# chenjiaoAngel/Paddle-Lite

Measured on AMD Instinct MI355X. Metric: INT8 images/sec MobileNetV1 224x224, higher is better.
Workload: dtype int8; 1 GPU; MobileNetV1 INT8 full graph 224x224 (27 int8 convs + pool + fc + softmax), random-init weights, 128 images per step and GPU (4 predictors / HIP streams, each running whole steps: 4 steps in flight), input resident in HBM; steps_in_flight=4, global_batch=128

## Files before the change

### paddle-lite_amd/csrc/fused_dwpw_stream.hip

```cpp
#include <stdlib.h>

#include <type_traits>

#include "plhip_device.h"
#include "plhip_kernels.h"
#include "dw_common.h"
#include "gemm_tr_common.h"

namespace plhip {

typedef float v2f __attribute__((ext_vector_type(2)));


constexpr int FS_STAMP_SLOTS = 8;

template <int W, int K, int M, int TP, int RS, int PD, int S, int MP, int OUT, bool DWNN, bool PWNN>
__global__ __launch_bounds__(256, M / MP >= 256 ? 2 : 3) void fused_dwpw_stream_kernel(FusedArgs a) {
  constexpr int FS_TP = TP, FS_NT = TP / 32, FS_PITCH = fs_pitch(TP);
  static_assert((FS_PITCH / 4) % 16 == 8 && FS_PITCH >= TP, "image pitch");
  constexpr int RP = (W + 3) / 4 * 4;
  constexpr int TR = W == 14 ? 7 : FS_TP / RP, NS = TR / RS, QW = RP / 4;
  static_assert(RP == W || (S == 2 && RP == 16), "partial quads: the stride-2 form only");
  constexpr int G = 64 / QW;
  constexpr int NGRP = K * NS;
  constexpr int NIT = (NGRP + 4 * G - 1) / (4 * G);
  constexpr int KS = K / 32, MT = M / 32 / MP;
  constexpr int MSPLIT = MT >= 4 ? 4 : MT;
  constexpr int NSPLIT = 4 / MSPLIT;
  constexpr int MW = MT / MSPLIT;
  constexpr int NW = (FS_NT + NSPLIT - 1) / NSPLIT;
  constexpr int NIN = S == 1 ? RS + 2 : 2 * RS + 1;
  constexpr int ND = S == 1 ? 2 : 3;
  constexpr int WI = S * W;
  static_assert(S == 1 || S == 2, "stride");
  static_assert(TR * RP <= FS_TP && TR % RS == 0 && K % 32 == 0 && M % (32 * MP) == 0 && MT % MSPLIT == 0, "geometry");
  const GemmArgs& g = a.pw;
  PLHIP_PRELOAD(a.x); PLHIP_PRELOAD(a.dw_w); PLHIP_PRELOAD(a.dw_scale); PLHIP_PRELOAD(a.dw_bias); PLHIP_PRELOAD(a.dw_act);
  PLHIP_PRELOAD(a.dw_alpha); PLHIP_PRELOAD(a.n); PLHIP_PRELOAD(a.h); PLHIP_PRELOAD(a.tiles); PLHIP_PRELOAD(a.ones); PLHIP_PRELOAD(g.wp);
  PLHIP_PRELOAD(g.y); PLHIP_PRELOAD(g.scale); PLHIP_PRELOAD(g.bias); PLHIP_PRELOAD(g.act); PLHIP_PRELOAD(g.alpha); PLHIP_PRELOAD(g.NT);
  extern __shared__ __attribute__((aligned(16))) uint8_t fs_lds[];
  const int lane = threadIdx.x & 63;
  const int wave = __builtin_amdgcn_readfirstlane(threadIdx.x >> 6);
  const unsigned nb = (unsigned)a.tiles, per = (nb + 7) >> 3;
  const unsigned vb = (blockIdx.x & 7) * per + (blockIdx.x >> 3);
  if (vb >= nb) return;
  const int H = a.oh, TPI = g.NT;
  const int b = (int)(vb / (unsigned)TPI), ti = (int)(vb - (unsigned)b * TPI), tr0 = ti * TR;
  const int c = lane & 31, h = lane >> 5;
  unsigned long long* const gstamp = PLHIP_STAMPS_OF(g);
  const bool diag = kStamps && gstamp && vb < 2048;
  unsigned long long* const lstamp = diag ? gstamp + ((size_t)vb * 4 + wave) * FS_STAMP_SLOTS : nullptr;
  PLHIP_STAMP_REAL(0);
  PLHIP_STAMP(1);

  const int gl = lane / QW, q = lane - gl * QW;
  const bool active = gl < G;
  const int colq = q == 0 ? 0 : (q == QW - 1 ? W - 8 : 4 * q - 1);
  const uint32_t sel_lo = q == 0 ? 0x0201000cu : (q == QW - 1 ? 0x06050403u : 0x03020100u);
  const uint32_t sel_hi = q == 0 ? 0x06050403u : (q == QW - 1 ? 0x0c0c0c07u : 0x07060504u);
  const float dw_hi2 = a.dw_act == ACT_RELU6 ? fminf(a.dw_alpha + a.dw_alpha, 254.f) : 254.f;
  const float dw_leak = a.dw_act == ACT_LEAKY ? a.dw_alpha : 1.f;
  const uint32_t plane = (uint32_t)H * W, plane_in = (uint32_t)a.h * WI;
  const uint32_t m0 = q == 0 ? 0xffffff00u : 0xffffffffu;
  constexpr bool OVER = RP > W;
  const int x_last = (int)((uint32_t)a.n * K * plane_in) - 12;

  uint32_t in[PD][NIN][ND];
  uint8_t* const prm = fs_lds + (size_t)K * FS_PITCH;
  static_assert(K <= 256, "one channel's parameters per thread");
  uint32_t pw0 = 0, pw1 = 0, pw2 = 0;
  float psc0 = 0.f, pbi0 = 0.f;
  if ((int)threadIdx.x < K) {
    const int8_t* wp = a.dw_w + (size_t)threadIdx.x * 9;
    __builtin_memcpy(&pw0, wp, 4);
    __builtin_memcpy(&pw1, wp + 3, 4);
    __builtin_memcpy(&pw2, wp + 5, 4);
    psc0 = a.dw_scale[threadIdx.x];
    pbi0 = (a.dw_bias ? a.dw_bias : a.dw_scale)[threadIdx.x];
  }
  auto task = [&](int it, int& ch, int& strip, int& r0) {
    int gi = (it * 4 + wave) * G + (active ? gl : 0);
    if (gi >= NGRP) gi = NGRP - 1;
    ch = gi / NS;
    strip = gi - ch * NS;
    r0 = tr0 + strip * RS;
    if (r0 > H - RS) r0 = H - RS;
  };
  using std::integral_constant;
  auto fetch = [&](auto it_c) __attribute__((always_inline)) {
    constexpr int it = decltype(it_c)::value, s = it % PD;
    int ch, strip, r0;
    task(it, ch, strip, r0);
    const uint8_t* xs = reinterpret_cast<const uint8_t*>(a.x);
    if constexpr (S == 1) {
      const uint32_t off0 = (uint32_t)(b * K + ch) * plane + (uint32_t)r0 * W + colq;
      const bool top = r0 == 0, bot = r0 + RS == H;
      __builtin_memcpy(in[s][0], xs + (top ? off0 : off0 - W), 8);
#pragma unroll
      for (int t = 1; t <= RS; ++t) __builtin_memcpy(in[s][t], xs + off0 + (t - 1) * W, 8);
      __builtin_memcpy(in[s][RS + 1], xs + (bot ? off0 + (RS - 1) * W : off0 + RS * W), 8);
    } else {
      const int off0 = (int)((uint32_t)(b * K + ch) * plane_in + (uint32_t)(2 * r0) * WI) + 8 * q - 4;
      const int o1 = off0 < 0 ? 0 : off0;
      __builtin_memcpy(in[s][0], xs + (r0 == 0 ? o1 : off0 - WI), 12);
      __builtin_memcpy(in[s][1], xs + o1, 12);
#pragma unroll
      for (int t = 2; t < NIN; ++t) {
        int o = off0 + (t - 1) * WI;
        if (OVER && t == NIN - 1) o = o > x_last ? x_last : o;
        __builtin_memcpy(in[s][t], xs + o, 12);
      }
    }
  };
  auto compute = [&](auto it_c) __attribute__((always_inline)) {
    constexpr int it = decltype(it_c)::value, s = it % PD;
    int ch, strip, r0;
    task(it, ch, strip, r0);
    const uint32_t zt = r0 == 0 ? 0u : 0xffffffffu, zb = r0 + RS == H ? 0u : 0xffffffffu;
    constexpr bool SINK = M / MP < 256;
    const uint32_t ldsa = (uint32_t)ch * FS_PITCH + (uint32_t)(strip * RS) * RP + 4 * q;
    const uint32_t ldsw = SINK && !active ? (uint32_t)(K * FS_PITCH + K * 32) + 4 * (lane & 7) : ldsa;
    int dacc[RS][4];
    const v4i pv = *reinterpret_cast<const v4i*>(prm + ch * 32);
    const uint32_t wr[3] = {(uint32_t)pv[0], (uint32_t)pv[1], (uint32_t)pv[2]};
    const uint32_t w0t = wr[0] & zt, w2b = S == 1 ? wr[2] & zb : wr[2];
    const uint32_t wu[3] = {wr[0] << 8, wr[1] << 8, wr[2] << 8};
    const uint32_t w0tu = w0t << 8;
    const bool fix = S == 2 && b == 0 && ch == 0 && q == 0 && r0 == 0;
    const bool fixe = OVER && b == a.n - 1 && ch == K - 1 && q == QW - 1 && r0 + RS == H;
    const float dsc = __uint_as_float((uint32_t)pv[3]), dbi = __uint_as_float(*reinterpret_cast<const uint32_t*>(prm + ch * 32 + 16));
#pragma unroll
    for (int t = 0; t < NIN; ++t) {
      uint32_t win[4];
      if constexpr (S == 1) {
        const uint32_t e0 = __builtin_amdgcn_perm(in[s][t][1], in[s][t][0], sel_lo), e1 = __builtin_amdgcn_perm(in[s][t][1], in[s][t][0], sel_hi);
        win[0] = e0;
        win[1] = __builtin_amdgcn_alignbyte(e1, e0, 1);
        win[2] = __builtin_amdgcn_alignbyte(e1, e0, 2);
        win[3] = __builtin_amdgcn_alignbyte(e1, e0, 3);
#pragma unroll
        for (int r = 0; r < 3; ++r) {
          const int o = t - r;
          if (o < 0 || o >= RS) continue;
#pragma unroll
          for (int jj = 0; jj < 4; ++jj)
            dacc[o][jj] = r == 0 ? sdot4_first(win[jj], t == 0 ? w0t : wr[0])
                                 : __builtin_amdgcn_sdot4((int)win[jj], (int)(t == NIN - 1 ? w2b : wr[r]), dacc[o][jj], false);
        }
      } else {
        uint32_t d0 = in[s][t][0], d1 = in[s][t][1], d2 = in[s][t][2];
        if (t < 2) {
          d2 = fix ? d1 : d2;
          d1 = fix ? d0 : d1;
        }
        if (OVER && t == NIN - 1) {
          d0 = fixe ? d1 : d0;
          d1 = fixe ? d2 : d1;
        }
        win[0] = __builtin_amdgcn_alignbyte(d1, d0, 3) & m0;
        win[1] = __builtin_amdgcn_alignbyte(d2, d1, 1);
        win[2] = __builtin_amdgcn_alignbyte(d2, d1, 3);
        win[3] = d2;
#pragma unroll
        for (int r = 0; r < 3; ++r) {
          if ((t - r) & 1) continue;
          const int o = (t - r) / 2;
          if (t - r < 0 || o >= RS) continue;
          const uint32_t f = t == 0 ? w0t : wr[r], fu = t == 0 ? w0tu : wu[r];
#pragma unroll
          for (int jj = 0; jj < 4; ++jj)
            dacc[o][jj] = r == 0 ? sdot4_first(win[jj], jj == 3 ? fu : f)
                                 : __builtin_amdgcn_sdot4((int)win[jj], (int)(jj == 3 ? fu : f), dacc[o][jj], false);
        }
      }
    }
#pragma unroll
    for (int o = 0; o < RS; ++o) {
      const uint32_t pk = DWNN ? requant4_nn_rtz(dacc[o], dsc, dbi, dw_hi2, a.ones)
                               : dw_requant4<ACT_LEAKY>(dacc[o], dsc, dbi, dw_leak, -254.f, 254.f);
      if (SINK || active) *reinterpret_cast<uint32_t*>(fs_lds + ldsw + o * RP) = pk;
    }
  };
  auto prime = [&](auto self, auto it_c) __attribute__((always_inline)) -> void {
    constexpr int it = decltype(it_c)::value;
    if constexpr (it < PD && it < NIT) {
      fetch(it_c);
      self(self, integral_constant<int, it + 1>{});
    }
  };
  prime(prime, integral_constant<int, 0>{});
  PLHIP_STAMP(2);
  const int ms = wave % MSPLIT, ns = wave / MSPLIT;
  const int n0 = ns * NW;
  const int nmine = n0 + NW <= FS_NT ? NW : FS_NT - n0;
  const uint32_t trb = (uint32_t)(((h * 2) * 8 + ((lane & 15) >> 1)) * FS_PITCH + ((lane >> 4) & 1) * 16 + (lane & 1) * 8 + n0 * 32);
  const uint32_t wlane = (uint32_t)lane * 16;
  constexpr int WBUDGET = 192, ACCR = NW * MW * 16;
  constexpr int WD = KS < 4 ? 2 : (ACCR + KS * MW * 4 <= WBUDGET ? KS : (ACCR + 4 * MW * 4 <= WBUDGET ? 4 : 2));
  constexpr int WPRE = WD == KS ? KS : WD - 1;
  constexpr bool ALOOK = M / MP >= 256 && NSPLIT == 1 && ACCR + WD * MW * 4 <= WBUDGET;
  v4i Wf[WD][MW];
  float psc[2][MW], pbi[2][MW];
  auto pass_w = [&](int mp) { return reinterpret_cast<const uint8_t*>(g.wp) + (size_t)((mp * MSPLIT + ms) * MW) * KS * 1024; };
  auto pass_operands = [&](auto mp_c) __attribute__((always_inline)) {
    constexpr int mp = decltype(mp_c)::value;
    const uint8_t* const wpk = pass_w(mp);
    const int mt0 = (mp * MSPLIT + ms) * MW;
#pragma unroll
    for (int u = 0; u < WPRE && u < KS; ++u)
#pragma unroll
      for (int m = 0; m < MW; ++m) Wf[u][m] = *reinterpret_cast<const v4i*>(wpk + ((size_t)m * KS + u) * 1024 + wlane);
#pragma unroll
    for (int m = 0; m < MW; ++m) {
      psc[mp & 1][m] = 1.f;
      pbi[mp & 1][m] = 0.f;
      if (OUT != OUT_I32) {
        psc[mp & 1][m] = g.scale[(mt0 + m) * 32 + c];
        pbi[mp & 1][m] = (g.bias ? g.bias : g.scale)[(mt0 + m) * 32 + c];
        if (!g.bias) pbi[mp & 1][m] = 0.f;
      }
    }
  };
  pass_operands(integral_constant<int, 0>{});
  if ((int)threadIdx.x < K) {
    uint32_t* o = reinterpret_cast<uint32_t*>(prm + threadIdx.x * 32);
    const v4i pv = {(int)(pw0 & 0xffffffu), (int)(pw1 & 0xffffffu), (int)(pw2 >> 8), (int)__float_as_uint(psc0 + psc0)};
    *reinterpret_cast<v4i*>(o) = pv;
    o[4] = a.dw_bias ? __float_as_uint(pbi0 + pbi0) : 0u;
  }
  __syncthreads();
  auto steps = [&](auto self, auto it_c) __attribute__((always_inline)) -> void {
    constexpr int it = decltype(it_c)::value;
    if constexpr (it < NIT) {
      compute(it_c);
      if constexpr (it + PD < NIT) fetch(integral_constant<int, it + PD>{});
      self(self, integral_constant<int, it + 1>{});
    }
  };
  steps(steps, integral_constant<int, 0>{});
  PLHIP_STAMP(3);
  __syncthreads();
  PLHIP_STAMP(4);

  const int vrows = H - tr0 < TR ? H - tr0 : TR;
  const int vpx = vrows * W;
  const float hi2 = g.act == ACT_RELU6 ? fminf(g.alpha + g.alpha, 254.f) : 254.f;
  const float leak = g.act == ACT_LEAKY ? g.alpha : 1.f;
  const float fcap = g.act == ACT_RELU6 ? g.alpha : __builtin_huge_valf();
  const float flo = (g.act == ACT_RELU || g.act == ACT_RELU6) ? 0.f : -__builtin_huge_valf();
  auto pass = [&](auto self, auto mp_c) __attribute__((always_inline)) -> void {
    constexpr int mp = decltype(mp_c)::value;
    if constexpr (mp < MP) {
      const uint8_t* const wpk = pass_w(mp);
      const int mt0 = (mp * MSPLIT + ms) * MW;
      v16i acc[NW][MW];
      const v16i zero16 = {0, 0, 0, 0, 0, 0, 0, 0, 0, 0, 0, 0, 0, 0, 0, 0};
      auto afrag = [&](int ks, int n) __attribute__((always_inline)) {
        const uint32_t ka = trb + (uint32_t)ks * (32 * FS_PITCH) + n * 32;
        const v2i lo = __builtin_amdgcn_ds_read_tr8_b64_v2i32((lds_v2i_ptr_t)(fs_lds + ka));
        const v2i hi = __builtin_amdgcn_ds_read_tr8_b64_v2i32((lds_v2i_ptr_t)(fs_lds + ka + 8 * FS_PITCH));
        const v4i av = {lo[0], lo[1], hi[0], hi[1]};
        return av;
      };
      constexpr int AL = 3;
      static_assert(!ALOOK || AL < KS * NW, "lookahead");
      v4i aq[AL + 1];
#pragma unroll
      for (int ks = 0; ks < KS; ++ks) {
        if (ks + WPRE < KS) {
#pragma unroll
          for (int m = 0; m < MW; ++m)
            Wf[(ks + WPRE) % WD][m] = *reinterpret_cast<const v4i*>(wpk + ((size_t)m * KS + ks + WPRE) * 1024 + wlane);
        }
#pragma unroll
        for (int n = 0; n < NW; ++n) {
          if (ALOOK || n < nmine) {
            v4i av;
            if constexpr (ALOOK) {
              const int i = ks * NW + n;
              if (i == 0) {
#pragma unroll
                for (int j = 0; j < AL; ++j) aq[j] = afrag(j / NW, j % NW);
              }
              if (i + AL < KS * NW) aq[(i + AL) % (AL + 1)] = afrag((i + AL) / NW, (i + AL) % NW);
              __builtin_amdgcn_sched_barrier(0);
              av = aq[i % (AL + 1)];
            } else {
              av = afrag(ks, n);
            }
#pragma unroll
            for (int m = 0; m < MW; ++m)
              acc[n][m] = __builtin_amdgcn_mfma_i32_32x32x32_i8(av, Wf[ks % WD][m], ks == 0 ? zero16 : acc[n][m], 0, 0, 0);
          }
        }
      }
      if constexpr (mp == MP - 1) PLHIP_STAMP(5);
      if constexpr (mp + 1 < MP) pass_operands(integral_constant<int, mp + 1>{});
#pragma unroll
      for (int m = 0; m < MW; ++m) {
        const int mch = (mt0 + m) * 32 + c;
        const float sc = psc[mp & 1][m], bi = pbi[mp & 1][m];
        const size_t obase = ((size_t)b * M + mch) * plane + (size_t)tr0 * W;
#pragma unroll
        for (int n = 0; n < NW; ++n) {
          if (n >= nmine) continue;
          const int px0 = (n0 + n) * 32;
          if (OUT == OUT_I8) {
            const float s2 = sc + sc, b2 = bi + bi;
            uint32_t edw[4];
#pragma unroll
            for (int gq = 0; gq < 4; ++gq) {
              int v[4] = {acc[n][m][4 * gq], acc[n][m][4 * gq + 1], acc[n][m][4 * gq + 2], acc[n][m][4 * gq + 3]};
              edw[gq] = PWNN ? requant4_nn_rtz(v, s2, b2, hi2, a.ones) : dw_requant4<ACT_LEAKY>(v, s2, b2, leak, -254.f, 254.f);
            }
            auto s02 = __builtin_amdgcn_permlane32_swap(edw[0], edw[2], false, false);
            auto s13 = __builtin_amdgcn_permlane32_swap(edw[1], edw[3], false, false);
            const int px = px0 + 16 * h;
            int8_t* const yo = reinterpret_cast<int8_t*>(g.y) + obase;
            if constexpr (RP == W) {
              const v4i v = {(int)s02[0], (int)s02[1], (int)s13[0], (int)s13[1]};
              if (px < vpx) *reinterpret_cast<v4i*>(yo + px) = v;
            } else {
              const int row = px >> 4;
              if (row < vrows) {
                int8_t* const yr = yo + row * W;
                const v2i v01 = {(int)s02[0], (int)s02[1]};
                __builtin_memcpy(yr, &v01, 8);
                const uint32_t v2 = s13[0];
                __builtin_memcpy(yr + 8, &v2, 4);
                const uint16_t v3 = (uint16_t)s13[1];
                __builtin_memcpy(yr + 12, &v3, 2);
              }
            }
          } else {
#pragma unroll
            for (int gq = 0; gq < 4; ++gq) {
              const int px = px0 + 8 * gq + 4 * h;
              int nval = 4;
              size_t opx = px;
              if constexpr (RP == W) {
                if (px >= vpx) continue;
              } else {
                const int row = px >> 4, col = px & 15;
                if (row >= vrows) continue;
                nval = col == 12 ? 2 : 4;
                opx = (size_t)row * W + col;
              }
              if (OUT == OUT_F32) {
                float f[4];
#pragma unroll
                for (int e = 0; e < 4; ++e) {
                  float y = __fmaf_rn((float)acc[n][m][4 * gq + e], sc, bi);
                  if (g.act == ACT_LEAKY) y = y > 0.f ? y : g.alpha * y;
                  f[e] = fminf(fmaxf(y, flo), fcap);
                }
                float* const yf = reinterpret_cast<float*>(g.y) + obase + opx;
                if (nval == 4) {
                  const v4f v = {f[0], f[1], f[2], f[3]};
                  __builtin_memcpy(yf, &v, 16);
                } else {
                  const v2f v = {f[0], f[1]};
                  __builtin_memcpy(yf, &v, 8);
                }
              } else {
                int* const yi = reinterpret_cast<int*>(g.y) + obase + opx;
                if (nval == 4) {
                  const v4i v = {acc[n][m][4 * gq], acc[n][m][4 * gq + 1], acc[n][m][4 * gq + 2], acc[n][m][4 * gq + 3]};
                  __builtin_memcpy(yi, &v, 16);
                } else {
                  const v2i v = {acc[n][m][4 * gq], acc[n][m][4 * gq + 1]};
                  __builtin_memcpy(yi, &v, 8);
                }
              }
            }
          }
        }
      }
      self(self, integral_constant<int, mp + 1>{});
    }
  };
  pass(pass, integral_constant<int, 0>{});
  PLHIP_STAMP(6);
  PLHIP_STAMP_REAL(7);
}

void run_fused_stream(const DwPlan& p, FusedArgs a, int out, hipStream_t s) {
  PLHIP_SET_STAMPS(a.pw, "fs", sizeof(unsigned long long) * 2048 * 4 * FS_STAMP_SLOTS);
  auto run = [&](auto shape) {
    constexpr dw_plan_detail::StreamShape T = dw_plan_detail::kStreamShapes[decltype(shape)::value];
    with_out_nonneg<OUT_I32, OUT_F32, OUT_I8>(out, a.dw_act, a.pw.act, [&](auto out_c, auto dn, auto pn) {
      launch_max_lds(fused_dwpw_stream_kernel<T.W, T.K, T.M, T.TP, T.RS, T.PD, T.S, T.MP, decltype(out_c)::value, decltype(dn)::value != 0,
                                              decltype(pn)::value != 0>, p, s, a);
    });
  };
  int i = 0;
  while (!(dw_plan_detail::kStreamShapes[i].W == p.W && dw_plan_detail::kStreamShapes[i].S == p.S)) ++i;
  with_const<0, 1, 2, 3, 4, 5>(i, run);
}

}
```

Measured before the change: 427,100 img/s.

## Skip dead strips on short tiles and block-wide item map in fused dw/pw kernel

Replaces the per-wave task mapping with a block-wide item map over all 256 threads, rotating the wave order by block index. For the last tile of an image, which has fewer valid rows, the depthwise loop runs a compile-time specialised, shorter iteration count, and waves with no live items skip their fetch and compute. The pointwise epilogue also skips 32-pixel column tiles beyond the valid pixels. This removes redundant depthwise work and stores on partial tiles, at the cost of instantiating two unrolled depthwise loops per kernel, which adds code size and register pressure.

```diff
diff --git a/paddle-lite_amd/csrc/fused_dwpw_stream.hip b/paddle-lite_amd/csrc/fused_dwpw_stream.hip
--- a/paddle-lite_amd/csrc/fused_dwpw_stream.hip
+++ b/paddle-lite_amd/csrc/fused_dwpw_stream.hip
@@ -6,6 +6,7 @@
 #include "plhip_kernels.h"
 #include "dw_common.h"
 #include "gemm_tr_common.h"
+#include "stream_items.h"
 
 namespace plhip {
 
@@ -21,9 +22,10 @@
   constexpr int RP = (W + 3) / 4 * 4;
   constexpr int TR = W == 14 ? 7 : FS_TP / RP, NS = TR / RS, QW = RP / 4;
   static_assert(RP == W || (S == 2 && RP == 16), "partial quads: the stride-2 form only");
-  constexpr int G = 64 / QW;
-  constexpr int NGRP = K * NS;
-  constexpr int NIT = (NGRP + 4 * G - 1) / (4 * G);
+  constexpr StreamItems IM = stream_items(dw_plan_detail::StreamShape{W, S, K, M, TP, RS, PD, MP});
+  static_assert(IM.RP == RP && IM.QW == QW && IM.TR == TR && IM.NS == NS, "item map");
+  constexpr int NVS_MIN = stream_valid_strips(IM, stream_min_vrows(IM, W));
+  static_assert(W % RS == 0 && NS <= 2, "whole strips; the item map divides by NS only");
   constexpr int KS = K / 32, MT = M / 32 / MP;
   constexpr int MSPLIT = MT >= 4 ? 4 : MT;
   constexpr int NSPLIT = 4 / MSPLIT;
@@ -53,8 +55,10 @@
   PLHIP_STAMP_REAL(0);
   PLHIP_STAMP(1);
 
-  const int gl = lane / QW, q = lane - gl * QW;
-  const bool active = gl < G;
+  const int vrows = H - tr0 < TR ? H - tr0 : TR;
+  const bool short_tile = NS > 1 && stream_valid_strips(IM, vrows) < NS;
+  const int pwave = wave ^ (int)(vb & 3), ptid = pwave * 64 + lane;
+  const int q = stream_item(IM, NS, 0, ptid).q;
   const int colq = q == 0 ? 0 : (q == QW - 1 ? W - 8 : 4 * q - 1);
   const uint32_t sel_lo = q == 0 ? 0x0201000cu : (q == QW - 1 ? 0x06050403u : 0x03020100u);
   const uint32_t sel_hi = q == 0 ? 0x06050403u : (q == QW - 1 ? 0x0c0c0c07u : 0x07060504u);
@@ -78,19 +82,24 @@
     psc0 = a.dw_scale[threadIdx.x];
     pbi0 = (a.dw_bias ? a.dw_bias : a.dw_scale)[threadIdx.x];
   }
-  auto task = [&](int it, int& ch, int& strip, int& r0) {
-    int gi = (it * 4 + wave) * G + (active ? gl : 0);
-    if (gi >= NGRP) gi = NGRP - 1;
-    ch = gi / NS;
-    strip = gi - ch * NS;
-    r0 = tr0 + strip * RS;
-    if (r0 > H - RS) r0 = H - RS;
+  auto task = [&](auto nvs_c, auto it_c, int& r0) __attribute__((always_inline)) {
+    constexpr int it = decltype(it_c)::value, nvs = decltype(nvs_c)::value;
+    StreamItem i = stream_item(IM, nvs, it, ptid);
+    if constexpr ((it + 1) * IM.GB <= K * nvs) i.live = ptid < IM.STRIDE;
+    r0 = tr0 + i.strip * RS;
+    return i;
+  };
+  auto wave_live = [&](auto nvs_c, auto it_c) __attribute__((always_inline)) {
+    constexpr int it = decltype(it_c)::value, nvs = decltype(nvs_c)::value;
+    if constexpr (stream_wave_live(IM, nvs, it, 3)) return true;
+    else return stream_wave_live(IM, nvs, it, pwave);
   };
   using std::integral_constant;
-  auto fetch = [&](auto it_c) __attribute__((always_inline)) {
+  auto fetch = [&](auto nvs_c, auto it_c) __attribute__((always_inline)) {
     constexpr int it = decltype(it_c)::value, s = it % PD;
-    int ch, strip, r0;
-    task(it, ch, strip, r0);
+    int r0;
+    const StreamItem item = task(nvs_c, it_c, r0);
+    const int ch = item.ch;
     const uint8_t* xs = reinterpret_cast<const uint8_t*>(a.x);
     if constexpr (S == 1) {
       const uint32_t off0 = (uint32_t)(b * K + ch) * plane + (uint32_t)r0 * W + colq;
@@ -112,13 +121,15 @@
       }
     }
   };
-  auto compute = [&](auto it_c) __attribute__((always_inline)) {
+  auto compute = [&](auto nvs_c, auto it_c) __attribute__((always_inline)) {
     constexpr int it = decltype(it_c)::value, s = it % PD;
-    int ch, strip, r0;
-    task(it, ch, strip, r0);
+    int r0;
+    const StreamItem item = task(nvs_c, it_c, r0);
+    const int ch = item.ch;
+    const bool active = item.live;
     const uint32_t zt = r0 == 0 ? 0u : 0xffffffffu, zb = r0 + RS == H ? 0u : 0xffffffffu;
     constexpr bool SINK = M / MP < 256;
-    const uint32_t ldsa = (uint32_t)ch * FS_PITCH + (uint32_t)(strip * RS) * RP + 4 * q;
+    const uint32_t ldsa = stream_item_lds(IM, FS_PITCH, item, 0);
     const uint32_t ldsw = SINK && !active ? (uint32_t)(K * FS_PITCH + K * 32) + 4 * (lane & 7) : ldsa;
     int dacc[RS][4];
     const v4i pv = *reinterpret_cast<const v4i*>(prm + ch * 32);
@@ -181,14 +192,17 @@
       if (SINK || active) *reinterpret_cast<uint32_t*>(fs_lds + ldsw + o * RP) = pk;
     }
   };
-  auto prime = [&](auto self, auto it_c) __attribute__((always_inline)) -> void {
+  auto prime = [&](auto self, auto nvs_c, auto it_c) __attribute__((always_inline)) -> void {
     constexpr int it = decltype(it_c)::value;
-    if constexpr (it < PD && it < NIT) {
-      fetch(it_c);
-      self(self, integral_constant<int, it + 1>{});
-    }
-  };
-  prime(prime, integral_constant<int, 0>{});
+    if constexpr (it < PD && it < stream_iterations(IM, decltype(nvs_c)::value)) {
+      if (wave_live(nvs_c, it_c)) fetch(nvs_c, it_c);
+      self(self, nvs_c, integral_constant<int, it + 1>{});
+    }
+  };
+  constexpr integral_constant<int, NS> full_c{};
+  constexpr integral_constant<int, NVS_MIN> short_c{};
+  if (short_tile) prime(prime, short_c, integral_constant<int, 0>{});
+  else prime(prime, full_c, integral_constant<int, 0>{});
   PLHIP_STAMP(2);
   const int ms = wave % MSPLIT, ns = wave / MSPLIT;
   const int n0 = ns * NW;
@@ -229,21 +243,28 @@
     o[4] = a.dw_bias ? __float_as_uint(pbi0 + pbi0) : 0u;
   }
   __syncthreads();
-  auto steps = [&](auto self, auto it_c) __attribute__((always_inline)) -> void {
-    constexpr int it = decltype(it_c)::value;
-    if constexpr (it < NIT) {
-      compute(it_c);
-      if constexpr (it + PD < NIT) fetch(integral_constant<int, it + PD>{});
-      self(self, integral_constant<int, it + 1>{});
-    }
-  };
-  steps(steps, integral_constant<int, 0>{});
+  auto steps = [&](auto self, auto nvs_c, auto it_c) __attribute__((always_inline)) -> void {
+    constexpr int it = decltype(it_c)::value, nit = stream_iterations(IM, decltype(nvs_c)::value);
+    if constexpr (it < nit) {
+      if (wave_live(nvs_c, it_c)) {
+        compute(nvs_c, it_c);
+        if constexpr (it + PD < nit) {
+          if (wave_live(nvs_c, integral_constant<int, it + PD>{})) fetch(nvs_c, integral_constant<int, it + PD>{});
+        }
+        self(self, nvs_c, integral_constant<int, it + 1>{});
+      }
+    }
+  };
+  if (short_tile) steps(steps, short_c, integral_constant<int, 0>{});
+  else steps(steps, full_c, integral_constant<int, 0>{});
   PLHIP_STAMP(3);
   __syncthreads();
   PLHIP_STAMP(4);
 
-  const int vrows = H - tr0 < TR ? H - tr0 : TR;
   const int vpx = vrows * W;
+  constexpr bool SHORT = W % TR != 0;
+  const int nv = SHORT ? (vpx + 31) >> 5 : FS_NT;
+  const int nvw = SHORT ? (nv - n0 < nmine ? nv - n0 : nmine) : nmine;
   const float hi2 = g.act == ACT_RELU6 ? fminf(g.alpha + g.alpha, 254.f) : 254.f;
   const float leak = g.act == ACT_LEAKY ? g.alpha : 1.f;
   const float fcap = g.act == ACT_RELU6 ? g.alpha : __builtin_huge_valf();
@@ -303,7 +324,7 @@
         const size_t obase = ((size_t)b * M + mch) * plane + (size_t)tr0 * W;
 #pragma unroll
         for (int n = 0; n < NW; ++n) {
-          if (n >= nmine) continue;
+          if (n >= nvw) continue;
           const int px0 = (n0 + n) * 32;
           if (OUT == OUT_I8) {
             const float s2 = sc + sc, b2 = bi + bi;
diff --git a/paddle-lite_amd/csrc/stream_items.h b/paddle-lite_amd/csrc/stream_items.h
--- /dev/null
+++ b/paddle-lite_amd/csrc/stream_items.h
@@ -0,0 +1,60 @@
+#pragma once
+#include "dw_plan.h"
+
+#if defined(__HIP__) || defined(__HIPCC__)
+#define PLHIP_ITEMS_FN __host__ __device__ constexpr inline
+#else
+#define PLHIP_ITEMS_FN constexpr inline
+#endif
+
+namespace plhip {
+
+constexpr int FS_THREADS = 256;
+
+struct StreamItems {
+  int K, RS;
+  int RP;
+  int QW;
+  int TR;
+  int NS;
+  int GB;
+  int STRIDE;
+};
+PLHIP_ITEMS_FN StreamItems stream_items(const dw_plan_detail::StreamShape& t) {
+  const int RP = (t.W + 3) / 4 * 4, QW = RP / 4, TR = t.W == 14 ? 7 : t.TP / RP;
+  return StreamItems{t.K, t.RS, RP, QW, TR, TR / t.RS, FS_THREADS / QW, FS_THREADS / QW * QW};
+}
+
+PLHIP_ITEMS_FN int stream_valid_strips(const StreamItems& m, int vrows) { return (vrows + m.RS - 1) / m.RS; }
+PLHIP_ITEMS_FN int stream_min_vrows(const StreamItems& m, int H) { return H % m.TR ? H % m.TR : m.TR; }
+PLHIP_ITEMS_FN int stream_item_count(const StreamItems& m, int nvs) { return m.K * nvs * m.QW; }
+PLHIP_ITEMS_FN int stream_iterations(const StreamItems& m, int nvs) { return (m.K * nvs + m.GB - 1) / m.GB; }
+PLHIP_ITEMS_FN bool stream_wave_live(const StreamItems& m, int nvs, int it, int wave) {
+  return 64 * wave < m.STRIDE && it * m.GB + 64 * wave / m.QW < m.K * nvs;
+}
+
+struct StreamItem {
+  int ch, strip, q;
+  bool live;
+};
+PLHIP_ITEMS_FN StreamItem stream_item(const StreamItems& m, int nvs, int it, int tid) {
+  const int gl = tid / m.QW, q = tid - gl * m.QW;
+  const int groups = m.K * nvs;
+  int gi = it * m.GB + gl;
+  const bool live = tid < m.STRIDE && gi < groups;
+  if (gi >= groups) gi = groups - 1;
+  int ch = gi, strip = 0;
+  if (m.NS == 1 || nvs == m.NS) {
+    ch = gi / m.NS;
+    strip = gi - ch * m.NS;
+  } else if (nvs != 1) {
+    ch = gi / nvs;
+    strip = gi - ch * nvs;
+  }
+  return StreamItem{ch, strip, q, live};
+}
+PLHIP_ITEMS_FN unsigned stream_item_lds(const StreamItems& m, int pitch, const StreamItem& i, int o) {
+  return (unsigned)i.ch * pitch + (unsigned)((i.strip * m.RS + o) * m.RP) + 4u * i.q;
+}
+
+}
```

After: 429,100 img/s (median of 6 runs). Within noise of the previous version (+0.5%).
